# NVIDIA-Merlin/distributed-embeddings

Measured on NVIDIA H100. Metric: DLRM global samples/sec (device-timed, max over ranks), higher is better.
Workload: dtype bf16

## Files before the change

distributed_embeddings_b200/ops/csrc/dense_kernels.cu:

```cuda
#include <cuda_bf16.h>
#include <cuda_runtime.h>
#include <stdint.h>

#include <cstdlib>

#include "common.cuh"
#include "de_b200.h"

namespace de {

namespace {

using bf16 = __nv_bfloat16;

__device__ __forceinline__ uint32_t smem_u32(const void* p) {
  return static_cast<uint32_t>(__cvta_generic_to_shared(p));
}

__device__ __forceinline__ void ldmatrix_x4(uint32_t (&r)[4], uint32_t addr) {
  asm volatile("ldmatrix.sync.aligned.m8n8.x4.shared.b16 {%0,%1,%2,%3}, [%4];"
               : "=r"(r[0]), "=r"(r[1]), "=r"(r[2]), "=r"(r[3])
               : "r"(addr));
}
__device__ __forceinline__ void ldmatrix_x4_trans(uint32_t (&r)[4], uint32_t addr) {
  asm volatile("ldmatrix.sync.aligned.m8n8.x4.trans.shared.b16 {%0,%1,%2,%3}, [%4];"
               : "=r"(r[0]), "=r"(r[1]), "=r"(r[2]), "=r"(r[3])
               : "r"(addr));
}
__device__ __forceinline__ void mma_bf16(float (&c)[4], const uint32_t (&a)[4], uint32_t b0,
                                         uint32_t b1) {
  asm volatile(
      "mma.sync.aligned.m16n8k16.row.col.f32.bf16.bf16.f32 {%0,%1,%2,%3}, {%4,%5,%6,%7}, "
      "{%8,%9}, {%0,%1,%2,%3};"
      : "+f"(c[0]), "+f"(c[1]), "+f"(c[2]), "+f"(c[3])
      : "r"(a[0]), "r"(a[1]), "r"(a[2]), "r"(a[3]), "r"(b0), "r"(b1));
}

constexpr int kMaxFeat = 32;
constexpr int kWarps = 4;

__host__ __device__ constexpr int fwd_warp_bytes(int d) {
  return (kMaxFeat * (d + 8) * 2 > kMaxFeat * 33 * 4) ? kMaxFeat * (d + 8) * 2 : kMaxFeat * 33 * 4;
}

__device__ __forceinline__ void cp_async16(void* smem_dst, const void* gmem_src) {
  asm volatile("cp.async.cg.shared.global [%0], [%1], 16;" ::"r"(smem_u32(smem_dst)),
               "l"(gmem_src)
               : "memory");
}
__device__ __forceinline__ void cp_async_wait_all() {
  asm volatile("cp.async.commit_group;\ncp.async.wait_group 0;" ::: "memory");
}

template <int D>
__device__ __forceinline__ void stage_features(bf16* sF, int LD, const bf16* bottom,
                                               const bf16* emb, int n_emb, int lane) {
  constexpr int kChunks = D / 8;
  const int total = (n_emb + 1) * kChunks;
#pragma unroll 4
  for (int c = lane; c < total; c += 32) {
    const int row = c / kChunks, ch = c - row * kChunks;
    const bf16* src = row == 0 ? bottom + ch * 8 : emb + (row - 1) * D + ch * 8;
    cp_async16(sF + row * LD + ch * 8, src);
  }
  cp_async_wait_all();
}

template <int D>
__device__ __forceinline__ void zero_pad_rows(bf16* sF, int LD, int n_emb, int lane) {
  constexpr int kChunks = D / 8;
  for (int c = (n_emb + 1) * kChunks + lane; c < kMaxFeat * kChunks; c += 32) {
    const int row = c / kChunks, ch = c - row * kChunks;
    *reinterpret_cast<uint4*>(sF + row * LD + ch * 8) = make_uint4(0, 0, 0, 0);
  }
}

template <int D>
__global__ void __launch_bounds__(kWarps * 32)
interact_fwd_kernel(const bf16* __restrict__ bottom, int64_t bottom_stride,
                    const bf16* __restrict__ emb, int64_t emb_stride, int n_emb,
                    bf16* __restrict__ z, int64_t z_stride, int z_width, int64_t batch,
                    const __grid_constant__ SyncArgs sync) {
  sync_head(sync);
  constexpr int LD = D + 8;
  constexpr int kWarpBytes = fwd_warp_bytes(D);
  extern __shared__ __align__(16) unsigned char smem_raw[];
  const int warp = threadIdx.x >> 5, lane = threadIdx.x & 31;
  bf16* sF = reinterpret_cast<bf16*>(smem_raw + warp * kWarpBytes);
  float* sC = reinterpret_cast<float*>(sF);
  const int nf = n_emb + 1;
  const int n_inter = nf * (nf - 1) / 2;

  for (int64_t s = static_cast<int64_t>(blockIdx.x) * kWarps + warp; s < batch;
       s += static_cast<int64_t>(gridDim.x) * kWarps) {
    const bf16* bp = bottom + s * bottom_stride;
    zero_pad_rows<D>(sF, LD, n_emb, lane);
    stage_features<D>(sF, LD, bp, emb + s * emb_stride, n_emb, lane);
    __syncwarp();
    float acc0[2][4] = {}, acc1[4][4] = {};
#pragma unroll
    for (int k = 0; k < D; k += 16) {
      uint32_t a0[4], a1[4], b01[4], b23[4];
      const int arow = lane & 15, acol = k + ((lane >> 4) << 3);
      ldmatrix_x4(a0, smem_u32(sF + arow * LD + acol));
      ldmatrix_x4(a1, smem_u32(sF + (16 + arow) * LD + acol));
      const int brow = (lane & 7) + ((lane >> 4) << 3), bcol = k + (((lane >> 3) & 1) << 3);
      ldmatrix_x4(b01, smem_u32(sF + brow * LD + bcol));
      ldmatrix_x4(b23, smem_u32(sF + (16 + brow) * LD + bcol));
      mma_bf16(acc0[0], a0, b01[0], b01[1]);
      mma_bf16(acc0[1], a0, b01[2], b01[3]);
      mma_bf16(acc1[0], a1, b01[0], b01[1]);
      mma_bf16(acc1[1], a1, b01[2], b01[3]);
      mma_bf16(acc1[2], a1, b23[0], b23[1]);
      mma_bf16(acc1[3], a1, b23[2], b23[3]);
    }
    __syncwarp();
    const int cr = lane >> 2, cc = (lane & 3) << 1;
#pragma unroll
    for (int nt = 0; nt < 2; ++nt) {
      sC[cr * 33 + nt * 8 + cc] = acc0[nt][0];
      sC[cr * 33 + nt * 8 + cc + 1] = acc0[nt][1];
      sC[(cr + 8) * 33 + nt * 8 + cc] = acc0[nt][2];
      sC[(cr + 8) * 33 + nt * 8 + cc + 1] = acc0[nt][3];
    }
#pragma unroll
    for (int nt = 0; nt < 4; ++nt) {
      sC[(16 + cr) * 33 + nt * 8 + cc] = acc1[nt][0];
      sC[(16 + cr) * 33 + nt * 8 + cc + 1] = acc1[nt][1];
      sC[(24 + cr) * 33 + nt * 8 + cc] = acc1[nt][2];
      sC[(24 + cr) * 33 + nt * 8 + cc + 1] = acc1[nt][3];
    }
    __syncwarp();
    bf16* zp = z + s * z_stride;
    for (int idx = lane; idx < n_inter; idx += 32) {
      int i = static_cast<int>((1.0f + sqrtf(1.0f + 8.0f * idx)) * 0.5f);
      while (i * (i - 1) / 2 > idx) --i;
      while ((i + 1) * i / 2 <= idx) ++i;
      const int j = idx - i * (i - 1) / 2;
      zp[idx] = __float2bfloat16_rn(sC[i * 33 + j]);
    }
    for (int c = lane; c < D; c += 32) zp[n_inter + c] = bp[c];
    for (int c = n_inter + D + lane; c < z_width; c += 32) zp[c] = __float2bfloat16_rn(0.f);
    __syncwarp();
  }
  sync_tail(sync);
}

template <int D>
__global__ void __launch_bounds__(kWarps * 32)
interact_bwd_kernel(const bf16* __restrict__ bottom, int64_t bottom_stride,
                    const bf16* __restrict__ emb, int64_t emb_stride, int n_emb,
                    const bf16* __restrict__ dz, int64_t dz_stride, bf16* __restrict__ dbottom,
                    int64_t dbottom_stride, bf16* __restrict__ demb, int64_t demb_stride,
                    float emb_grad_scale, int64_t batch) {
  constexpr int LD = D + 8;
  constexpr int LDG = 40;
  extern __shared__ __align__(16) unsigned char smem_raw[];
  const int warp = threadIdx.x >> 5, lane = threadIdx.x & 31;
  bf16* sF = reinterpret_cast<bf16*>(smem_raw) + warp * (kMaxFeat * LD + kMaxFeat * LDG);
  bf16* sG = sF + kMaxFeat * LD;
  const int nf = n_emb + 1;
  const int n_inter = nf * (nf - 1) / 2;
  zero_pad_rows<D>(sF, LD, n_emb, lane);

  for (int64_t s = static_cast<int64_t>(blockIdx.x) * kWarps + warp; s < batch;
       s += static_cast<int64_t>(gridDim.x) * kWarps) {
    stage_features<D>(sF, LD, bottom + s * bottom_stride, emb + s * emb_stride, n_emb, lane);
    const bf16* dzp = dz + s * dz_stride;
    for (int c = lane; c < kMaxFeat * LDG / 8; c += 32)
      reinterpret_cast<uint4*>(sG)[c] = make_uint4(0, 0, 0, 0);
    __syncwarp();
    for (int idx = lane; idx < n_inter; idx += 32) {
      int i = static_cast<int>((1.0f + sqrtf(1.0f + 8.0f * idx)) * 0.5f);
      while (i * (i - 1) / 2 > idx) --i;
      while ((i + 1) * i / 2 <= idx) ++i;
      const int j = idx - i * (i - 1) / 2;
      const bf16 v = dzp[idx];
      sG[i * LDG + j] = v;
      sG[j * LDG + i] = v;
    }
    __syncwarp();
    uint32_t ga[2][2][4];
#pragma unroll
    for (int mt = 0; mt < 2; ++mt)
#pragma unroll
      for (int ks = 0; ks < 2; ++ks)
        ldmatrix_x4(ga[mt][ks],
                    smem_u32(sG + (mt * 16 + (lane & 15)) * LDG + ks * 16 + ((lane >> 4) << 3)));
    const int cr = lane >> 2, cc = (lane & 3) << 1;
    bf16* dbp = dbottom + s * dbottom_stride;
    bf16* dep = demb + s * demb_stride;
#pragma unroll 1
    for (int n0 = 0; n0 < D; n0 += 32) {
      float acc[2][4][4] = {};
#pragma unroll
      for (int ks = 0; ks < 2; ++ks) {
        uint32_t b01[4], b23[4];
        const int krow = ks * 16 + (lane & 7) + (((lane >> 3) & 1) << 3);
        const int ncol = n0 + ((lane >> 4) << 3);
        ldmatrix_x4_trans(b01, smem_u32(sF + krow * LD + ncol));
        ldmatrix_x4_trans(b23, smem_u32(sF + krow * LD + ncol + 16));
#pragma unroll
        for (int mt = 0; mt < 2; ++mt) {
          mma_bf16(acc[mt][0], ga[mt][ks], b01[0], b01[1]);
          mma_bf16(acc[mt][1], ga[mt][ks], b01[2], b01[3]);
          mma_bf16(acc[mt][2], ga[mt][ks], b23[0], b23[1]);
          mma_bf16(acc[mt][3], ga[mt][ks], b23[2], b23[3]);
        }
      }
#pragma unroll
      for (int mt = 0; mt < 2; ++mt) {
#pragma unroll
        for (int nt = 0; nt < 4; ++nt) {
#pragma unroll
          for (int half = 0; half < 2; ++half) {
            const int row = mt * 16 + cr + half * 8;
            const int col = n0 + nt * 8 + cc;
            float v0 = acc[mt][nt][half * 2], v1 = acc[mt][nt][half * 2 + 1];
            if (row == 0) {
              v0 += __bfloat162float(dzp[n_inter + col]);
              v1 += __bfloat162float(dzp[n_inter + col + 1]);
              *reinterpret_cast<__nv_bfloat162*>(dbp + col) = __floats2bfloat162_rn(v0, v1);
            } else if (row <= n_emb) {
              *reinterpret_cast<__nv_bfloat162*>(dep + (row - 1) * D + col) =
                  __floats2bfloat162_rn(v0 * emb_grad_scale, v1 * emb_grad_scale);
            }
          }
        }
      }
    }
    __syncwarp();
  }
}

__device__ __forceinline__ void cp_async_commit() {
  asm volatile("cp.async.commit_group;" ::: "memory");
}
template <int N>
__device__ __forceinline__ void cp_async_wait_group() {
  asm volatile("cp.async.wait_group %0;" ::"n"(N) : "memory");
}

constexpr int kDzMax = 512;

template <int D>
__device__ __forceinline__ void issue_sample(bf16* sF, int LD, bf16* sDz, const bf16* bottom,
                                             const bf16* emb, const bf16* dz, int n_emb,
                                             int dz_chunks, int lane) {
  constexpr int kChunks = D / 8;
  const int total = (n_emb + 1) * kChunks;
#pragma unroll 4
  for (int c = lane; c < total; c += 32) {
    const int row = c / kChunks, ch = c - row * kChunks;
    const bf16* src = row == 0 ? bottom + ch * 8 : emb + (row - 1) * D + ch * 8;
    cp_async16(sF + row * LD + ch * 8, src);
  }
  for (int c = lane; c < dz_chunks; c += 32) cp_async16(sDz + c * 8, dz + c * 8);
}

struct ChunkDst {
  unsigned long long base;
  long long stride;
};

__device__ __forceinline__ void prefetch_l2(const void* p) {
  asm volatile("prefetch.global.L2 [%0];" ::"l"(p));
}

template <int D, bool APPLY>
__device__ __forceinline__ void
interact_bwd_v2_body(const bf16* __restrict__ bottom, int64_t bottom_stride,
                     const bf16* __restrict__ emb, int64_t emb_stride, int n_emb,
                     const bf16* __restrict__ dz, int64_t dz_stride, bf16* __restrict__ dbottom,
                     int64_t dbottom_stride, bf16* __restrict__ demb, int64_t demb_stride,
                     float emb_grad_scale, int64_t batch, const GradRoute* __restrict__ routes,
                     int n_routes, const SyncArgs& sync, uint32_t* __restrict__ done_counters,
                     int chunk_rows, const InteractApply& apply) {
  constexpr int LD = D + 8;
  constexpr int LDG = 40;
  constexpr int kWarpElems = 2 * kMaxFeat * LD + 2 * kDzMax + kMaxFeat * LDG;
  constexpr int kRowChunks = D / 8;
  extern __shared__ __align__(16) unsigned char smem_raw[];
  const int warp = threadIdx.x >> 5, lane = threadIdx.x & 31;
  bf16* base = reinterpret_cast<bf16*>(smem_raw) + warp * kWarpElems;
  bf16* sDz0 = base + 2 * kMaxFeat * LD;
  bf16* sG = sDz0 + 2 * kDzMax;
  ChunkDst* sDst = reinterpret_cast<ChunkDst*>(reinterpret_cast<bf16*>(smem_raw) +
                                               kWarps * kWarpElems);
  const int nf = n_emb + 1;
  const int n_inter = nf * (nf - 1) / 2;
  const int dz_chunks = (n_inter + D + 7) >> 3;
  const int n_chunks = n_emb * kRowChunks;
  if (routes == nullptr) {
    for (int c = threadIdx.x; c < n_chunks; c += blockDim.x) {
      sDst[c].base = reinterpret_cast<unsigned long long>(demb + c * 8);
      sDst[c].stride = demb_stride * 2;
    }
  } else {
    for (int r = 0; r < n_routes; ++r) {
      const GradRoute R = routes[r];
      const int c0 = R.src_col >> 3, nc = R.width >> 3;
      for (int c = threadIdx.x; c < nc; c += blockDim.x) {
        sDst[c0 + c].base =
            reinterpret_cast<unsigned long long>(reinterpret_cast<bf16*>(R.dst) + R.dst_col + c * 8);
        sDst[c0 + c].stride = R.dst_stride * 2;
      }
    }
  }
  zero_pad_rows<D>(base, LD, n_emb, lane);
  zero_pad_rows<D>(base + kMaxFeat * LD, LD, n_emb, lane);
  __syncthreads();

  float apply_scale = 0.f;
  long long id_cur = -1, id_next = -1;
  if constexpr (APPLY) {
    apply_scale = apply.scale;
    if (apply.scale_ptr != nullptr) apply_scale *= *apply.scale_ptr;
  }
  auto load_id = [&](int64_t smp) -> long long {
    if (lane < n_emb && ((apply.mask >> lane) & 1u)) {
      const long long raw = apply.ids64 ? static_cast<const int64_t*>(apply.ids[lane])[smp]
                                        : static_cast<const int32_t*>(apply.ids[lane])[smp];
      const long long id = raw + apply.id_shift[lane];
      if (static_cast<unsigned long long>(id) < static_cast<unsigned long long>(apply.sub_rows[lane]))
        return id;
    }
    return -1;
  };
  auto prefetch_row = [&](long long id) {
    if (id >= 0) {
      const char* row = reinterpret_cast<const char*>(apply.table[lane] +
                                                      (apply.row_base[lane] + id) * D);
#pragma unroll
      for (int l = 0; l < D * 4 / 128; ++l) prefetch_l2(row + (l << 7));
    }
  };

  const int64_t stride = static_cast<int64_t>(gridDim.x) * kWarps;
  int64_t s = static_cast<int64_t>(blockIdx.x) * kWarps + warp;
  int cur = 0;
  if (s < batch) {
    issue_sample<D>(base, LD, sDz0, bottom + s * bottom_stride, emb + s * emb_stride,
                    dz + s * dz_stride, n_emb, dz_chunks, lane);
    if constexpr (APPLY) {
      id_cur = load_id(s);
      prefetch_row(id_cur);
    }
  }
  cp_async_commit();
  for (; s < batch; s += stride, cur ^= 1) {
    const int64_t nxt = s + stride;
    if (nxt < batch) {
      issue_sample<D>(base + (cur ^ 1) * (kMaxFeat * LD), LD, sDz0 + (cur ^ 1) * kDzMax,
                      bottom + nxt * bottom_stride, emb + nxt * emb_stride, dz + nxt * dz_stride,
                      n_emb, dz_chunks, lane);
      if constexpr (APPLY) id_next = load_id(nxt);
    } else if constexpr (APPLY) {
      id_next = -1;
    }
    cp_async_commit();
    cp_async_wait_group<1>();
    __syncwarp();
    bf16* sF = base + cur * (kMaxFeat * LD);
    const bf16* sDz = sDz0 + cur * kDzMax;
    for (int c = lane; c < kMaxFeat * LDG / 8; c += 32)
      reinterpret_cast<uint4*>(sG)[c] = make_uint4(0, 0, 0, 0);
    __syncwarp();
    for (int idx = lane; idx < n_inter; idx += 32) {
      int i = static_cast<int>((1.0f + sqrtf(1.0f + 8.0f * idx)) * 0.5f);
      while (i * (i - 1) / 2 > idx) --i;
      while ((i + 1) * i / 2 <= idx) ++i;
      const int j = idx - i * (i - 1) / 2;
      const bf16 v = sDz[idx];
      sG[i * LDG + j] = v;
      sG[j * LDG + i] = v;
    }
    __syncwarp();
    uint32_t ga[2][2][4];
#pragma unroll
    for (int mt = 0; mt < 2; ++mt)
#pragma unroll
      for (int ks = 0; ks < 2; ++ks)
        ldmatrix_x4(ga[mt][ks],
                    smem_u32(sG + (mt * 16 + (lane & 15)) * LDG + ks * 16 + ((lane >> 4) << 3)));
    const int cr = lane >> 2, cc = (lane & 3) << 1;
#pragma unroll 1
    for (int n0 = 0; n0 < D; n0 += 32) {
      float acc[2][4][4] = {};
#pragma unroll
      for (int ks = 0; ks < 2; ++ks) {
        uint32_t b01[4], b23[4];
        const int krow = ks * 16 + (lane & 7) + (((lane >> 3) & 1) << 3);
        const int ncol = n0 + ((lane >> 4) << 3);
        ldmatrix_x4_trans(b01, smem_u32(sF + krow * LD + ncol));
        ldmatrix_x4_trans(b23, smem_u32(sF + krow * LD + ncol + 16));
#pragma unroll
        for (int mt = 0; mt < 2; ++mt) {
          mma_bf16(acc[mt][0], ga[mt][ks], b01[0], b01[1]);
          mma_bf16(acc[mt][1], ga[mt][ks], b01[2], b01[3]);
          mma_bf16(acc[mt][2], ga[mt][ks], b23[0], b23[1]);
          mma_bf16(acc[mt][3], ga[mt][ks], b23[2], b23[3]);
        }
      }
#pragma unroll
      for (int mt = 0; mt < 2; ++mt) {
#pragma unroll
        for (int nt = 0; nt < 4; ++nt) {
#pragma unroll
          for (int half = 0; half < 2; ++half) {
            const int row = mt * 16 + cr + half * 8;
            const int col = n0 + nt * 8 + cc;
            float v0 = acc[mt][nt][half * 2], v1 = acc[mt][nt][half * 2 + 1];
            if (row == 0) {
              v0 += __bfloat162float(sDz[n_inter + col]);
              v1 += __bfloat162float(sDz[n_inter + col + 1]);
            } else {
              v0 *= emb_grad_scale;
              v1 *= emb_grad_scale;
            }
            if (row <= n_emb)
              *reinterpret_cast<__nv_bfloat162*>(sF + row * LD + col) =
                  __floats2bfloat162_rn(v0, v1);
          }
        }
      }
    }
    __syncwarp();
    if constexpr (APPLY) prefetch_row(id_next);
    if (lane < kRowChunks)
      *reinterpret_cast<uint4*>(dbottom + s * dbottom_stride + lane * 8) =
          *reinterpret_cast<const uint4*>(sF + lane * 8);
    if constexpr (APPLY) {
      for (int c0 = 0; c0 < n_chunks; c0 += 32) {
        const int c = c0 + lane;
        const int f = c / kRowChunks, ch = c - f * kRowChunks;
        const long long id = __shfl_sync(0xffffffffu, id_cur, f & 31);
        if (c >= n_chunks) continue;
        const uint4 v = *reinterpret_cast<const uint4*>(sF + (f + 1) * LD + ch * 8);
        if ((apply.mask >> f) & 1u) {
          if (id >= 0) {
            const __nv_bfloat162* h = reinterpret_cast<const __nv_bfloat162*>(&v);
            FVec<4> lo, hi;
#pragma unroll
            for (int k = 0; k < 2; ++k) {
              const float2 a = __bfloat1622float2(h[k]), b = __bfloat1622float2(h[k + 2]);
              lo.v[2 * k] = a.x * apply_scale;
              lo.v[2 * k + 1] = a.y * apply_scale;
              hi.v[2 * k] = b.x * apply_scale;
              hi.v[2 * k + 1] = b.y * apply_scale;
            }
            float* dst = apply.table[f] + (apply.row_base[f] + id) * D + ch * 8;
            red_add_f32<4>(dst, lo);
            red_add_f32<4>(dst + 4, hi);
          }
        } else {
          const ChunkDst d = sDst[c];
          *reinterpret_cast<uint4*>(d.base + static_cast<unsigned long long>(s * d.stride)) = v;
        }
      }
      id_cur = id_next;
    } else {
      for (int c = lane; c < n_chunks; c += 32) {
        const int row = 1 + c / kRowChunks, ch = c - (row - 1) * kRowChunks;
        const ChunkDst d = sDst[c];
        *reinterpret_cast<uint4*>(d.base + static_cast<unsigned long long>(s * d.stride)) =
            *reinterpret_cast<const uint4*>(sF + row * LD + ch * 8);
      }
    }
    __syncwarp();
    if (done_counters != nullptr && lane == 0) {
      __threadfence();
      atomicAdd(done_counters + s / chunk_rows, 1u);
    }
  }
  cp_async_wait_group<0>();
  sync_tail(sync);
}

template <int D>
__global__ void __launch_bounds__(kWarps * 32)
interact_bwd_v2_kernel(const bf16* __restrict__ bottom, int64_t bottom_stride,
                       const bf16* __restrict__ emb, int64_t emb_stride, int n_emb,
                       const bf16* __restrict__ dz, int64_t dz_stride, bf16* __restrict__ dbottom,
                       int64_t dbottom_stride, bf16* __restrict__ demb, int64_t demb_stride,
                       float emb_grad_scale, int64_t batch,
                       const GradRoute* __restrict__ routes, int n_routes,
                       const __grid_constant__ SyncArgs sync, uint32_t* __restrict__ done_counters,
                       int chunk_rows) {
  interact_bwd_v2_body<D, false>(bottom, bottom_stride, emb, emb_stride, n_emb, dz, dz_stride,
                                 dbottom, dbottom_stride, demb, demb_stride, emb_grad_scale, batch,
                                 routes, n_routes, sync, done_counters, chunk_rows,
                                 InteractApply{});
}

template <int D>
__global__ void __launch_bounds__(kWarps * 32)
interact_bwd_apply_kernel(const bf16* __restrict__ bottom, int64_t bottom_stride,
                          const bf16* __restrict__ emb, int64_t emb_stride, int n_emb,
                          const bf16* __restrict__ dz, int64_t dz_stride,
                          bf16* __restrict__ dbottom, int64_t dbottom_stride,
                          bf16* __restrict__ demb, int64_t demb_stride, float emb_grad_scale,
                          int64_t batch, const GradRoute* __restrict__ routes, int n_routes,
                          const __grid_constant__ SyncArgs sync,
                          const __grid_constant__ InteractApply apply) {
  interact_bwd_v2_body<D, true>(bottom, bottom_stride, emb, emb_stride, n_emb, dz, dz_stride,
                                dbottom, dbottom_stride, demb, demb_stride, emb_grad_scale, batch,
                                routes, n_routes, sync, nullptr, 0, apply);
}

constexpr int kRbUnroll = 4;
__global__ void __launch_bounds__(256)
relu_bwd_bias_kernel(bf16* __restrict__ dy, const bf16* __restrict__ y, float* __restrict__ db,
                     int64_t rows, int cols, int rows_per_block) {
  extern __shared__ float s_part[];
  const int tpr = cols >> 3;
  const int rows_par = blockDim.x / tpr;
  const int tr = threadIdx.x / tpr, tc = threadIdx.x - tr * tpr;
  const int64_t r0 = static_cast<int64_t>(blockIdx.x) * rows_per_block;
  const int64_t r1 = min(rows, r0 + rows_per_block);
  float acc[8] = {0, 0, 0, 0, 0, 0, 0, 0};
  if (tr < rows_par) {
    for (int64_t r = r0 + tr; r < r1; r += static_cast<int64_t>(rows_par) * kRbUnroll) {
      uint4 g[kRbUnroll], a[kRbUnroll];
#pragma unroll
      for (int u = 0; u < kRbUnroll; ++u) {
        const int64_t rr = r + static_cast<int64_t>(u) * rows_par;
        if (rr < r1) {
          g[u] = *reinterpret_cast<const uint4*>(dy + rr * cols + tc * 8);
          a[u] = *reinterpret_cast<const uint4*>(y + rr * cols + tc * 8);
        }
      }
#pragma unroll
      for (int u = 0; u < kRbUnroll; ++u) {
        const int64_t rr = r + static_cast<int64_t>(u) * rows_par;
        if (rr < r1) {
          uint32_t* gw = reinterpret_cast<uint32_t*>(&g[u]);
          const uint32_t* aw = reinterpret_cast<const uint32_t*>(&a[u]);
#pragma unroll
          for (int i = 0; i < 4; ++i) {
            float2 gf = __bfloat1622float2(*reinterpret_cast<__nv_bfloat162*>(&gw[i]));
            const float2 af = __bfloat1622float2(*reinterpret_cast<const __nv_bfloat162*>(&aw[i]));
            gf.x = af.x > 0.f ? gf.x : 0.f;
            gf.y = af.y > 0.f ? gf.y : 0.f;
            acc[2 * i] += gf.x;
            acc[2 * i + 1] += gf.y;
            __nv_bfloat162 h = __floats2bfloat162_rn(gf.x, gf.y);
            gw[i] = *reinterpret_cast<uint32_t*>(&h);
          }
          *reinterpret_cast<uint4*>(dy + rr * cols + tc * 8) = g[u];
        }
      }
    }
#pragma unroll
    for (int i = 0; i < 8; ++i) s_part[tr * cols + tc * 8 + i] = acc[i];
  }
  __syncthreads();
  for (int c = threadIdx.x; c < cols; c += blockDim.x) {
    float v = 0.f;
    for (int t = 0; t < rows_par; ++t) v += s_part[t * cols + c];
    atomicAdd(db + c, v);
  }
}

__device__ __forceinline__ void unpack8(const uint4& v, float (&f)[8]) {
  const uint32_t* w = reinterpret_cast<const uint32_t*>(&v);
#pragma unroll
  for (int i = 0; i < 4; ++i) {
    const float2 t = unpack2<bf16>(w[i]);
    f[2 * i] = t.x;
    f[2 * i + 1] = t.y;
  }
}
__device__ __forceinline__ uint4 pack8(const float (&f)[8]) {
  uint4 v;
  uint32_t* w = reinterpret_cast<uint32_t*>(&v);
#pragma unroll
  for (int i = 0; i < 4; ++i) w[i] = pack2<bf16>(f[2 * i], f[2 * i + 1]);
  return v;
}

__global__ void __launch_bounds__(256)
cross_fwd_kernel(const uint4* __restrict__ x0, const uint4* __restrict__ s,
                 const uint4* __restrict__ xl, uint4* __restrict__ out, int64_t n_vec) {
  for (int64_t i = static_cast<int64_t>(blockIdx.x) * blockDim.x + threadIdx.x; i < n_vec;
       i += static_cast<int64_t>(gridDim.x) * blockDim.x) {
    float a[8], b[8], c[8];
    unpack8(x0[i], a);
    unpack8(s[i], b);
    unpack8(xl[i], c);
#pragma unroll
    for (int k = 0; k < 8; ++k) c[k] = fmaf(a[k], b[k], c[k]);
    out[i] = pack8(c);
  }
}


__global__ void __launch_bounds__(256)
cross_bwd_kernel(const bf16* __restrict__ dy, const bf16* __restrict__ x0, bf16* __restrict__ g,
                 float* __restrict__ db, int64_t rows, int cols, int tile, int rows_per_block) {
  extern __shared__ float s_part[];
  const int tpr = cols >> 3;
  const int v0 = blockIdx.y * tile;
  const int tw = min(tile, tpr - v0);
  const int rows_par = blockDim.x / tile;
  const int tr = threadIdx.x / tile, tc = threadIdx.x - tr * tile;
  const int64_t r0 = static_cast<int64_t>(blockIdx.x) * rows_per_block;
  const int64_t r1 = min(rows, r0 + rows_per_block);
  float acc[8] = {0, 0, 0, 0, 0, 0, 0, 0};
  const bool active = tr < rows_par && tc < tw;
  if (active) {
    const int64_t col = static_cast<int64_t>(v0 + tc) * 8;
    for (int64_t r = r0 + tr; r < r1; r += static_cast<int64_t>(rows_par) * kRbUnroll) {
      uint4 a[kRbUnroll], b[kRbUnroll];
#pragma unroll
      for (int u = 0; u < kRbUnroll; ++u) {
        const int64_t rr = r + static_cast<int64_t>(u) * rows_par;
        if (rr < r1) {
          a[u] = *reinterpret_cast<const uint4*>(dy + rr * cols + col);
          b[u] = *reinterpret_cast<const uint4*>(x0 + rr * cols + col);
        }
      }
#pragma unroll
      for (int u = 0; u < kRbUnroll; ++u) {
        const int64_t rr = r + static_cast<int64_t>(u) * rows_par;
        if (rr < r1) {
          float fa[8], fb[8];
          unpack8(a[u], fa);
          unpack8(b[u], fb);
#pragma unroll
          for (int k = 0; k < 8; ++k) {
            fa[k] *= fb[k];
            acc[k] += fa[k];
          }
          *reinterpret_cast<uint4*>(g + rr * cols + col) = pack8(fa);
        }
      }
    }
  }
  if (tr < rows_par) {
#pragma unroll
    for (int k = 0; k < 8; ++k) s_part[tr * tile * 8 + tc * 8 + k] = acc[k];
  }
  __syncthreads();
  for (int c = threadIdx.x; c < tw * 8; c += blockDim.x) {
    float v = 0.f;
    for (int t = 0; t < rows_par; ++t) v += s_part[t * tile * 8 + c];
    atomicAdd(db + v0 * 8 + c, v);
  }
}

__global__ void __launch_bounds__(256)
cross_dx0_kernel(const bf16* __restrict__ d_chain, const __grid_constant__ CrossTerms terms,
                 bf16* __restrict__ dx0, bf16* __restrict__ d_bottom, int64_t rows, int cols,
                 int emb_cols, int tile, int rows_per_block) {
  const int tpr = cols >> 3;
  const int v0 = blockIdx.y * tile;
  const int tw = min(tile, tpr - v0);
  const int rows_par = blockDim.x / tile;
  const int tr = threadIdx.x / tile, tc = threadIdx.x - tr * tile;
  if (tr >= rows_par || tc >= tw) return;
  const int col = (v0 + tc) * 8;
  const int64_t r0 = static_cast<int64_t>(blockIdx.x) * rows_per_block;
  const int64_t r1 = min(rows, r0 + rows_per_block);
  const int bcols = cols - emb_cols;
  bf16* dst = col < emb_cols ? dx0 + col : d_bottom + (col - emb_cols);
  const int64_t dst_stride = col < emb_cols ? cols : bcols;
  for (int64_t r = r0 + tr; r < r1; r += rows_par) {
    const int64_t off = r * cols + col;
    float acc[8];
    unpack8(*reinterpret_cast<const uint4*>(d_chain + off), acc);
    for (int l = 0; l < terms.n; ++l) {
      float a[8], b[8];
      unpack8(*(reinterpret_cast<const uint4*>(terms.dy[l]) + off / 8), a);
      unpack8(*(reinterpret_cast<const uint4*>(terms.s[l]) + off / 8), b);
#pragma unroll
      for (int k = 0; k < 8; ++k) acc[k] = fmaf(a[k], b[k], acc[k]);
    }
    *reinterpret_cast<uint4*>(dst + r * dst_stride) = pack8(acc);
  }
}

template <int PL>
__global__ void __launch_bounds__(256)
head_loss_kernel(const bf16* __restrict__ x, int K, const bf16* __restrict__ w,
                 const bf16* __restrict__ bias, const float* __restrict__ labels, int64_t batch,
                 float inv_batch, bf16* __restrict__ dx, float* __restrict__ dw,
                 float* __restrict__ db, float* __restrict__ dbias_prev,
                 float* __restrict__ loss_sum, float* __restrict__ logits_out) {
  extern __shared__ float sred[];
  float* s_dw = sred;
  float* s_dbp = sred + K;
  float* s_misc = sred + 2 * K;
  for (int i = threadIdx.x; i < 2 * K + 2; i += blockDim.x) sred[i] = 0.f;
  __syncthreads();
  const int warp = threadIdx.x >> 5, lane = threadIdx.x & 31;
  const int wpb = blockDim.x >> 5;
  constexpr int per_lane = PL;
  const float b0 = __bfloat162float(bias[0]);
  float wreg[PL];
#pragma unroll
  for (int i = 0; i < PL; ++i) wreg[i] = __bfloat162float(w[lane + 32 * i]);
  float dw_acc[PL], dbp_acc[PL];
#pragma unroll
  for (int i = 0; i < PL; ++i) dw_acc[i] = dbp_acc[i] = 0.f;
  float loss_acc = 0.f, db_acc = 0.f;
  for (int64_t s = static_cast<int64_t>(blockIdx.x) * wpb + warp; s < batch;
       s += static_cast<int64_t>(gridDim.x) * wpb) {
    float xv[PL];
    float dot = 0.f;
#pragma unroll
    for (int i = 0; i < PL; ++i) {
      if (i < per_lane) {
        xv[i] = __bfloat162float(x[s * K + lane + 32 * i]);
        dot = fmaf(xv[i], wreg[i], dot);
      }
    }
#pragma unroll
    for (int off = 16; off > 0; off >>= 1) dot += __shfl_xor_sync(0xffffffffu, dot, off);
    const float logit = dot + b0;
    const float label = labels[s];
    const float loss = fmaxf(logit, 0.f) - logit * label + log1pf(__expf(-fabsf(logit)));
    const float sig = 1.f / (1.f + __expf(-logit));
    const float dl = (sig - label) * inv_batch;
    if (lane == 0) {
      loss_acc += loss;
      db_acc += dl;
      if (logits_out) logits_out[s] = logit;
    }
#pragma unroll
    for (int i = 0; i < PL; ++i) {
      if (i < per_lane) {
        dw_acc[i] = fmaf(dl, xv[i], dw_acc[i]);
        const float g = xv[i] > 0.f ? dl * wreg[i] : 0.f;
        dbp_acc[i] += g;
        dx[s * K + lane + 32 * i] = __float2bfloat16_rn(g);
      }
    }
  }
#pragma unroll
  for (int i = 0; i < PL; ++i) {
    if (i < per_lane) {
      atomicAdd(&s_dw[lane + 32 * i], dw_acc[i]);
      atomicAdd(&s_dbp[lane + 32 * i], dbp_acc[i]);
    }
  }
  if (lane == 0) {
    atomicAdd(&s_misc[0], loss_acc);
    atomicAdd(&s_misc[1], db_acc);
  }
  __syncthreads();
  for (int i = threadIdx.x; i < K; i += blockDim.x) {
    atomicAdd(dw + i, s_dw[i]);
    atomicAdd(dbias_prev + i, s_dbp[i]);
  }
  if (threadIdx.x == 0) {
    atomicAdd(loss_sum, s_misc[0] * inv_batch);
    atomicAdd(db, s_misc[1]);
  }
}

template <int PL>
__global__ void __launch_bounds__(256)
head_eval_kernel(const bf16* __restrict__ x, const bf16* __restrict__ w,
                 const bf16* __restrict__ bias, const float* __restrict__ labels, int64_t batch,
                 const int64_t* __restrict__ n_valid, float* __restrict__ probs,
                 unsigned long long* __restrict__ hist, int nb, double* __restrict__ loss_sum,
                 unsigned long long* __restrict__ count) {
  constexpr int K = 32 * PL;
  __shared__ float s_loss;
  if (threadIdx.x == 0) s_loss = 0.f;
  __syncthreads();
  const int warp = threadIdx.x >> 5, lane = threadIdx.x & 31;
  const int wpb = blockDim.x >> 5;
  int64_t nv = *n_valid;
  nv = nv < 0 ? 0 : (nv > batch ? batch : nv);
  const float b0 = __bfloat162float(bias[0]);
  const float nbf = static_cast<float>(nb);
  float wreg[PL];
#pragma unroll
  for (int i = 0; i < PL; ++i) wreg[i] = __bfloat162float(w[lane + 32 * i]);
  float loss_acc = 0.f;
  for (int64_t g0 = (static_cast<int64_t>(blockIdx.x) * wpb + warp) * 32; g0 < batch;
       g0 += static_cast<int64_t>(gridDim.x) * wpb * 32) {
    const int rows = batch - g0 < 32 ? static_cast<int>(batch - g0) : 32;
    float my_logit = 0.f;
#pragma unroll 4
    for (int j = 0; j < rows; ++j) {
      const bf16* xr = x + (g0 + j) * K;
      float dot = 0.f;
#pragma unroll
      for (int i = 0; i < PL; ++i) dot = fmaf(__bfloat162float(xr[lane + 32 * i]), wreg[i], dot);
#pragma unroll
      for (int off = 16; off > 0; off >>= 1) dot += __shfl_xor_sync(0xffffffffu, dot, off);
      if (lane == j) my_logit = dot + b0;
    }
    const int64_t s = g0 + lane;
    const bool has_row = lane < rows;
    const bool valid = s < nv;
    const float logit = my_logit;
    const float p = 1.f / (1.f + __expf(-logit));
    if (has_row) probs[s] = p;
    int key = -1;
    if (valid) {
      const float label = labels[s];
      loss_acc += fmaxf(logit, 0.f) - logit * label + log1pf(__expf(-fabsf(logit)));
      int k = static_cast<int>(ceilf(__fmul_rn(p, nbf))) - 1;
      k = k < 0 ? 0 : (k > nb - 1 ? nb - 1 : k);
      key = (label > 0.5f ? nb : 0) + k;
    }
    const unsigned peers = __match_any_sync(0xffffffffu, key);
    if (key >= 0 && lane == __ffs(peers) - 1)
      atomicAdd(hist + key, static_cast<unsigned long long>(__popc(peers)));
  }
#pragma unroll
  for (int off = 16; off > 0; off >>= 1) loss_acc += __shfl_xor_sync(0xffffffffu, loss_acc, off);
  if (lane == 0) atomicAdd(&s_loss, loss_acc);
  __syncthreads();
  if (threadIdx.x == 0) {
    atomicAdd(loss_sum, static_cast<double>(s_loss));
    if (blockIdx.x == 0) atomicAdd(count, static_cast<unsigned long long>(nv));
  }
}

__global__ void __launch_bounds__(256)
sgd_update_kernel(float* __restrict__ p32, bf16* __restrict__ p16, float* __restrict__ g32,
                  const float* __restrict__ lr_ptr, float grad_scale, int64_t n_vec4) {
  const float step = -(*lr_ptr) * grad_scale;
  const int64_t stride = static_cast<int64_t>(gridDim.x) * blockDim.x;
  for (int64_t i = static_cast<int64_t>(blockIdx.x) * blockDim.x + threadIdx.x; i < n_vec4;
       i += stride) {
    float4 p = reinterpret_cast<float4*>(p32)[i];
    const float4 g = reinterpret_cast<const float4*>(g32)[i];
    p.x = fmaf(step, g.x, p.x);
    p.y = fmaf(step, g.y, p.y);
    p.z = fmaf(step, g.z, p.z);
    p.w = fmaf(step, g.w, p.w);
    reinterpret_cast<float4*>(p32)[i] = p;
    reinterpret_cast<float4*>(g32)[i] = make_float4(0.f, 0.f, 0.f, 0.f);
    __nv_bfloat162 a = __floats2bfloat162_rn(p.x, p.y), b = __floats2bfloat162_rn(p.z, p.w);
    uint2 o;
    o.x = *reinterpret_cast<uint32_t*>(&a);
    o.y = *reinterpret_cast<uint32_t*>(&b);
    reinterpret_cast<uint2*>(p16)[i] = o;
  }
}

template <int KIND>
__device__ __forceinline__ void dense_opt_elem(float& p, float& a, float& v, float g, float lr,
                                               float beta1, float beta2, float bias1, float bias2,
                                               float eps) {
  if constexpr (KIND == kOptAdagrad) {
    a = fmaf(g, g, a);
    p -= lr * g / (sqrtf(a) + eps);
  } else {
    a = beta1 * a + (1.f - beta1) * g;
    v = beta2 * v + (1.f - beta2) * g * g;
    const float mh = a / bias1;
    const float vh = v / bias2;
    p -= lr * mh / (sqrtf(vh) + eps);
  }
}

template <int KIND>
__global__ void __launch_bounds__(256)
dense_opt_kernel(float* __restrict__ p32, bf16* __restrict__ p16, float* __restrict__ g32,
                 float* __restrict__ s0, float* __restrict__ s1, const float* __restrict__ lr_ptr,
                 const float* __restrict__ step_ptr, float beta1, float beta2, float eps,
                 int64_t n_vec4) {
  const float lr = *lr_ptr;
  float bias1 = 1.f, bias2 = 1.f;
  if constexpr (KIND == kOptAdam) {
    const float t = *step_ptr;
    bias1 = 1.f - powf(beta1, t);
    bias2 = 1.f - powf(beta2, t);
  }
  const int64_t stride = static_cast<int64_t>(gridDim.x) * blockDim.x;
  for (int64_t i = static_cast<int64_t>(blockIdx.x) * blockDim.x + threadIdx.x; i < n_vec4;
       i += stride) {
    float4 p = reinterpret_cast<float4*>(p32)[i];
    const float4 g = reinterpret_cast<const float4*>(g32)[i];
    float4 a = reinterpret_cast<float4*>(s0)[i];
    float4 v = make_float4(0.f, 0.f, 0.f, 0.f);
    if constexpr (KIND == kOptAdam) v = reinterpret_cast<float4*>(s1)[i];
    dense_opt_elem<KIND>(p.x, a.x, v.x, g.x, lr, beta1, beta2, bias1, bias2, eps);
    dense_opt_elem<KIND>(p.y, a.y, v.y, g.y, lr, beta1, beta2, bias1, bias2, eps);
    dense_opt_elem<KIND>(p.z, a.z, v.z, g.z, lr, beta1, beta2, bias1, bias2, eps);
    dense_opt_elem<KIND>(p.w, a.w, v.w, g.w, lr, beta1, beta2, bias1, bias2, eps);
    reinterpret_cast<float4*>(p32)[i] = p;
    reinterpret_cast<float4*>(s0)[i] = a;
    if constexpr (KIND == kOptAdam) reinterpret_cast<float4*>(s1)[i] = v;
    reinterpret_cast<float4*>(g32)[i] = make_float4(0.f, 0.f, 0.f, 0.f);
    __nv_bfloat162 lo = __floats2bfloat162_rn(p.x, p.y), hi = __floats2bfloat162_rn(p.z, p.w);
    uint2 o;
    o.x = *reinterpret_cast<uint32_t*>(&lo);
    o.y = *reinterpret_cast<uint32_t*>(&hi);
    reinterpret_cast<uint2*>(p16)[i] = o;
  }
}

__global__ void cast_pad_kernel(const float* __restrict__ src, int src_cols, bf16* __restrict__ dst,
                                int dst_cols, int64_t rows) {
  const int64_t n = rows * dst_cols;
  const int64_t stride = static_cast<int64_t>(gridDim.x) * blockDim.x;
  for (int64_t i = static_cast<int64_t>(blockIdx.x) * blockDim.x + threadIdx.x; i < n;
       i += stride) {
    const int64_t r = i / dst_cols;
    const int c = static_cast<int>(i - r * dst_cols);
    dst[i] = __float2bfloat16_rn(c < src_cols ? src[r * src_cols + c] : 0.f);
  }
}

__global__ void __launch_bounds__(256)
avgpool_fwd_kernel(const bf16* __restrict__ x, int64_t x_stride, int n, bf16* __restrict__ out,
                   int64_t out_stride, int out_len, int stride, int left, int64_t rows) {
  const int64_t total = rows * out_len;
  const int64_t step = static_cast<int64_t>(gridDim.x) * blockDim.x;
  for (int64_t i = static_cast<int64_t>(blockIdx.x) * blockDim.x + threadIdx.x; i < total;
       i += step) {
    const int64_t r = i / out_len;
    const int j = static_cast<int>(i - r * out_len);
    const int lo = max(0, j * stride - left), hi = min(n, (j + 1) * stride - left);
    const bf16* xp = x + r * x_stride;
    float acc = 0.f;
    for (int c = lo; c < hi; ++c) acc += __bfloat162float(xp[c]);
    out[r * out_stride + j] = __float2bfloat16_rn(hi > lo ? acc / static_cast<float>(hi - lo) : 0.f);
  }
}

__global__ void __launch_bounds__(256)
avgpool_bwd_kernel(const bf16* __restrict__ dout, int64_t dout_stride, int out_len,
                   bf16* __restrict__ dx, int64_t dx_stride, int n, int stride, int left,
                   int64_t rows) {
  const int64_t total = rows * n;
  const int64_t step = static_cast<int64_t>(gridDim.x) * blockDim.x;
  for (int64_t i = static_cast<int64_t>(blockIdx.x) * blockDim.x + threadIdx.x; i < total;
       i += step) {
    const int64_t r = i / n;
    const int c = static_cast<int>(i - r * n);
    const int j = (c + left) / stride;
    const int lo = max(0, j * stride - left), hi = min(n, (j + 1) * stride - left);
    const float g = j < out_len ? __bfloat162float(dout[r * dout_stride + j]) : 0.f;
    dx[r * dx_stride + c] = __float2bfloat16_rn(g / static_cast<float>(hi - lo));
  }
}

}

void launch_avgpool_fwd(const void* x, int64_t x_stride, int n, void* out, int64_t out_stride,
                        int out_len, int stride, int left, int64_t rows, cudaStream_t stream) {
  if (rows <= 0 || out_len <= 0) return;
  int64_t blocks = (rows * out_len + 255) / 256;
  if (blocks > kGridCapSms * 16) blocks = kGridCapSms * 16;
  avgpool_fwd_kernel<<<static_cast<unsigned>(blocks), 256, 0, stream>>>(
      reinterpret_cast<const bf16*>(x), x_stride, n, reinterpret_cast<bf16*>(out), out_stride,
      out_len, stride, left, rows);
}

void launch_avgpool_bwd(const void* dout, int64_t dout_stride, int out_len, void* dx,
                        int64_t dx_stride, int n, int stride, int left, int64_t rows,
                        cudaStream_t stream) {
  if (rows <= 0 || n <= 0) return;
  int64_t blocks = (rows * n + 255) / 256;
  if (blocks > kGridCapSms * 16) blocks = kGridCapSms * 16;
  avgpool_bwd_kernel<<<static_cast<unsigned>(blocks), 256, 0, stream>>>(
      reinterpret_cast<const bf16*>(dout), dout_stride, out_len, reinterpret_cast<bf16*>(dx),
      dx_stride, n, stride, left, rows);
}

bool launch_interact_fwd(const void* bottom, int64_t bottom_stride, const void* emb,
                         int64_t emb_stride, int n_emb, int dim, void* z, int64_t z_stride,
                         int z_width, int64_t batch, int sm_count, cudaStream_t stream,
                         const SyncArgs& sync) {
  if (n_emb + 1 > kMaxFeat || batch <= 0) return false;
  int64_t blocks = (batch + kWarps - 1) / kWarps;
  const int64_t cap = static_cast<int64_t>(sm_count) * 8;
  if (blocks > cap) blocks = cap;
#define DE_IFWD(DD)                                                                              \
  {                                                                                              \
    const size_t smem = kWarps * fwd_warp_bytes(DD);                                             \
    cudaFuncSetAttribute(interact_fwd_kernel<DD>, cudaFuncAttributeMaxDynamicSharedMemorySize,   \
                         static_cast<int>(smem));                                                \
    interact_fwd_kernel<DD><<<static_cast<unsigned>(blocks), kWarps * 32, smem, stream>>>(       \
        reinterpret_cast<const bf16*>(bottom), bottom_stride, reinterpret_cast<const bf16*>(emb), \
        emb_stride, n_emb, reinterpret_cast<bf16*>(z), z_stride, z_width, batch, sync);          \
    return true;                                                                                 \
  }
  if (dim == 128) DE_IFWD(128)
  if (dim == 64) DE_IFWD(64)
  if (dim == 32) DE_IFWD(32)
  if (dim == 16) DE_IFWD(16)
#undef DE_IFWD
  return false;
}

bool launch_interact_bwd(const void* bottom, int64_t bottom_stride, const void* emb,
                         int64_t emb_stride, int n_emb, int dim, const void* dz,
                         int64_t dz_stride, void* dbottom, int64_t dbottom_stride, void* demb,
                         int64_t demb_stride, float emb_grad_scale, int64_t batch, int sm_count,
                         cudaStream_t stream, const GradRoute* routes, int n_routes,
                         const SyncArgs& sync, uint32_t* done_counters, int chunk_rows,
                         const InteractApply* apply) {
  if (n_emb + 1 > kMaxFeat || batch <= 0 || dim % 32 != 0) return false;
  const bool applied = apply != nullptr && apply->mask != 0;
  if (applied && (dim != 128 || done_counters != nullptr)) return false;
  int64_t blocks = (batch + kWarps - 1) / kWarps;
  const int64_t cap = static_cast<int64_t>(sm_count) * 8;
  if (blocks > cap) blocks = cap;
  static const bool force_v1 = [] {
    const char* v = std::getenv("DE_B200_INTERACT_V1");
    return v != nullptr && v[0] == '1';
  }();
  const int nf = n_emb + 1;
  const int dz_elems = (nf * (nf - 1) / 2 + dim + 7) / 8 * 8;
  const bool v2_ok =
      dz_elems <= kDzMax && dz_elems <= dz_stride && dz_stride % 8 == 0 &&
      bottom_stride % 8 == 0 && emb_stride % 8 == 0 && dbottom_stride % 8 == 0 &&
      ((reinterpret_cast<uintptr_t>(dz) | reinterpret_cast<uintptr_t>(bottom) |
        reinterpret_cast<uintptr_t>(emb) | reinterpret_cast<uintptr_t>(dbottom)) & 15) == 0 &&
      (dim == 128 || dim == 64) &&
      (routes != nullptr || (demb_stride % 8 == 0 && (reinterpret_cast<uintptr_t>(demb) & 15) == 0));
  if ((routes != nullptr || done_counters != nullptr || applied) && !v2_ok) return false;
  const bool has_sync = sync.state != nullptr && (sync.wait_ch >= 0 || sync.signal_ch >= 0);
  if (v2_ok &&
      (!force_v1 || routes != nullptr || has_sync || done_counters != nullptr || applied)) {
    int64_t blocks2 = (batch + kWarps - 1) / kWarps;
    if (blocks2 > static_cast<int64_t>(sm_count) * 2) blocks2 = static_cast<int64_t>(sm_count) * 2;
#define DE_IBWD2(KERNEL, DD, ...)                                                                \
  {                                                                                              \
    const size_t smem =                                                                          \
        kWarps * (2 * kMaxFeat * (DD + 8) + 2 * kDzMax + kMaxFeat * 40) * sizeof(bf16) +         \
        static_cast<size_t>(n_emb) * (DD / 8) * sizeof(ChunkDst);                                \
    cudaFuncSetAttribute(KERNEL<DD>, cudaFuncAttributeMaxDynamicSharedMemorySize,                \
                         static_cast<int>(smem));                                                \
    KERNEL<DD><<<static_cast<unsigned>(blocks2), kWarps * 32, smem, stream>>>(                   \
        reinterpret_cast<const bf16*>(bottom), bottom_stride, reinterpret_cast<const bf16*>(emb), \
        emb_stride, n_emb, reinterpret_cast<const bf16*>(dz), dz_stride,                         \
        reinterpret_cast<bf16*>(dbottom), dbottom_stride, reinterpret_cast<bf16*>(demb),         \
        demb_stride, emb_grad_scale, batch, routes, n_routes, sync, __VA_ARGS__);                \
    return true;                                                                                 \
  }
    if (applied) DE_IBWD2(interact_bwd_apply_kernel, 128, *apply)
    if (dim == 128) DE_IBWD2(interact_bwd_v2_kernel, 128, done_counters, chunk_rows)
    if (dim == 64) DE_IBWD2(interact_bwd_v2_kernel, 64, done_counters, chunk_rows)
#undef DE_IBWD2
  }
  if (has_sync) return false;
#define DE_IBWD(DD)                                                                              \
  {                                                                                              \
    const size_t smem = kWarps * (kMaxFeat * (DD + 8) + kMaxFeat * 40) * sizeof(bf16);           \
    cudaFuncSetAttribute(interact_bwd_kernel<DD>, cudaFuncAttributeMaxDynamicSharedMemorySize,   \
                         static_cast<int>(smem));                                                \
    interact_bwd_kernel<DD><<<static_cast<unsigned>(blocks), kWarps * 32, smem, stream>>>(       \
        reinterpret_cast<const bf16*>(bottom), bottom_stride, reinterpret_cast<const bf16*>(emb), \
        emb_stride, n_emb, reinterpret_cast<const bf16*>(dz), dz_stride,                         \
        reinterpret_cast<bf16*>(dbottom), dbottom_stride, reinterpret_cast<bf16*>(demb),         \
        demb_stride, emb_grad_scale, batch);                                                     \
    return true;                                                                                 \
  }
  if (dim == 128) DE_IBWD(128)
  if (dim == 64) DE_IBWD(64)
  if (dim == 32) DE_IBWD(32)
#undef DE_IBWD
  return false;
}

static void cross_tiling(int cols, int* tile, int* n_tiles, int* rows_per_block) {
  const int tpr = cols / 8;
  int best_t = 0, best_n = 0;
  double best = -1.0;
  for (int n = (tpr + 255) / 256; n <= tpr && n <= 64; ++n) {
    const int t = (tpr + n - 1) / n;
    const int rows_par = 256 / t;
    const double busy = static_cast<double>(rows_par * t) / 256.0 *
                        static_cast<double>(tpr) / static_cast<double>(n * t);
    if (busy > best + 1e-9) {
      best = busy;
      best_t = t;
      best_n = n;
    }
  }
  *tile = best_t;
  *n_tiles = best_n;
  *rows_per_block = (256 / best_t) * kRbUnroll * 4;
}

void launch_cross_fwd(const void* x0, const void* s, const void* xl, void* out, int64_t n,
                      int sm_count, cudaStream_t stream) {
  const int64_t n_vec = n / 8;
  if (n_vec <= 0) return;
  int64_t blocks = (n_vec + 255) / 256;
  if (blocks > sm_count * 8) blocks = sm_count * 8;
  cross_fwd_kernel<<<static_cast<unsigned>(blocks), 256, 0, stream>>>(
      reinterpret_cast<const uint4*>(x0), reinterpret_cast<const uint4*>(s),
      reinterpret_cast<const uint4*>(xl), reinterpret_cast<uint4*>(out), n_vec);
}

void launch_cross_bwd(const void* dy, const void* x0, void* g, float* db, int64_t rows, int cols,
                      cudaStream_t stream) {
  if (rows <= 0) return;
  int tile, n_tiles, rpb;
  cross_tiling(cols, &tile, &n_tiles, &rpb);
  const dim3 grid(static_cast<unsigned>((rows + rpb - 1) / rpb), static_cast<unsigned>(n_tiles));
  const size_t smem = static_cast<size_t>(256 / tile) * tile * 8 * sizeof(float);
  cross_bwd_kernel<<<grid, 256, smem, stream>>>(
      reinterpret_cast<const bf16*>(dy), reinterpret_cast<const bf16*>(x0),
      reinterpret_cast<bf16*>(g), db, rows, cols, tile, rpb);
}

void launch_cross_dx0(const void* d_chain, const CrossTerms& terms, void* dx0, void* d_bottom,
                      int64_t rows, int cols, int emb_cols, cudaStream_t stream) {
  if (rows <= 0) return;
  int tile, n_tiles, rpb;
  cross_tiling(cols, &tile, &n_tiles, &rpb);
  const dim3 grid(static_cast<unsigned>((rows + rpb - 1) / rpb), static_cast<unsigned>(n_tiles));
  cross_dx0_kernel<<<grid, 256, 0, stream>>>(
      reinterpret_cast<const bf16*>(d_chain), terms, reinterpret_cast<bf16*>(dx0),
      reinterpret_cast<bf16*>(d_bottom), rows, cols, emb_cols, tile, rpb);
}

void launch_relu_bwd_bias(void* dy, const void* y, float* db, int64_t rows, int cols,
                          cudaStream_t stream) {
  if (rows <= 0) return;
  const int tpr = cols / 8;
  const int threads = 256;
  const int rows_par = threads / tpr;
  const int rows_per_block = rows_par * kRbUnroll * 4;
  const int64_t blocks = (rows + rows_per_block - 1) / rows_per_block;
  const size_t smem = static_cast<size_t>(rows_par) * cols * sizeof(float);
  relu_bwd_bias_kernel<<<static_cast<unsigned>(blocks), threads, smem, stream>>>(
      reinterpret_cast<bf16*>(dy), reinterpret_cast<const bf16*>(y), db, rows, cols,
      rows_per_block);
}

bool launch_head_loss(const void* x, int K, const void* w, const void* bias, const float* labels,
                      int64_t batch, float inv_batch, void* dx, float* dw, float* db,
                      float* dbias_prev, float* loss_sum, float* logits_out, int sm_count,
                      cudaStream_t stream) {
  if (batch <= 0) return true;
  const int threads = 256;
  int64_t blocks = (batch + 7) / 8;
  if (blocks > sm_count * 4) blocks = sm_count * 4;
  const size_t smem = (2 * K + 2) * sizeof(float);
#define DE_HEAD(PL)                                                                              \
  head_loss_kernel<PL><<<static_cast<unsigned>(blocks), threads, smem, stream>>>(                \
      reinterpret_cast<const bf16*>(x), K, reinterpret_cast<const bf16*>(w),                     \
      reinterpret_cast<const bf16*>(bias), labels, batch, inv_batch, reinterpret_cast<bf16*>(dx), \
      dw, db, dbias_prev, loss_sum, logits_out)
  switch (K) {
    case 64: DE_HEAD(2); break;
    case 128: DE_HEAD(4); break;
    case 256: DE_HEAD(8); break;
    case 512: DE_HEAD(16); break;
    case 1024: DE_HEAD(32); break;
    default: return false;
  }
#undef DE_HEAD
  return true;
}

bool launch_head_eval(const void* x, int K, const void* w, const void* bias, const float* labels,
                      int64_t batch, const int64_t* n_valid, float* probs, int64_t* hist, int nb,
                      double* loss_sum, int64_t* count, int sm_count, cudaStream_t stream) {
  if (K != 64 && K != 128 && K != 256 && K != 512 && K != 1024) return false;
  if (batch <= 0) return true;
  const int threads = 256;
  int64_t blocks = (batch + 255) / 256;
  if (blocks > sm_count * 4) blocks = sm_count * 4;
#define DE_HEAD_EVAL(PL)                                                                         \
  head_eval_kernel<PL><<<static_cast<unsigned>(blocks), threads, 0, stream>>>(                  \
      reinterpret_cast<const bf16*>(x), reinterpret_cast<const bf16*>(w),                        \
      reinterpret_cast<const bf16*>(bias), labels, batch, n_valid, probs,                        \
      reinterpret_cast<unsigned long long*>(hist), nb, loss_sum,                                 \
      reinterpret_cast<unsigned long long*>(count))
  switch (K) {
    case 64: DE_HEAD_EVAL(2); break;
    case 128: DE_HEAD_EVAL(4); break;
    case 256: DE_HEAD_EVAL(8); break;
    case 512: DE_HEAD_EVAL(16); break;
    default: DE_HEAD_EVAL(32); break;
  }
#undef DE_HEAD_EVAL
  return true;
}

void launch_sgd_update(float* p32, void* p16, float* g32, const float* lr_ptr, float grad_scale,
                       int64_t n, int sm_count, cudaStream_t stream) {
  const int64_t n_vec4 = n / 4;
  if (n_vec4 <= 0) return;
  int64_t blocks = (n_vec4 + 255) / 256;
  if (blocks > sm_count * 8) blocks = sm_count * 8;
  sgd_update_kernel<<<static_cast<unsigned>(blocks), 256, 0, stream>>>(
      p32, reinterpret_cast<bf16*>(p16), g32, lr_ptr, grad_scale, n_vec4);
}

bool launch_dense_opt(int kind, float* p32, void* p16, float* g32, float* s0, float* s1,
                      const float* lr_ptr, const float* step_ptr, float beta1, float beta2,
                      float eps, int64_t n, int sm_count, cudaStream_t stream) {
  if (kind != kOptAdagrad && kind != kOptAdam) return false;
  const int64_t n_vec4 = n / 4;
  if (n_vec4 <= 0) return true;
  int64_t blocks = (n_vec4 + 255) / 256;
  if (blocks > sm_count * 8) blocks = sm_count * 8;
  if (kind == kOptAdagrad)
    dense_opt_kernel<kOptAdagrad><<<static_cast<unsigned>(blocks), 256, 0, stream>>>(
        p32, reinterpret_cast<bf16*>(p16), g32, s0, nullptr, lr_ptr, nullptr, 0.f, 0.f, eps,
        n_vec4);
  else
    dense_opt_kernel<kOptAdam><<<static_cast<unsigned>(blocks), 256, 0, stream>>>(
        p32, reinterpret_cast<bf16*>(p16), g32, s0, s1, lr_ptr, step_ptr, beta1, beta2, eps,
        n_vec4);
  return true;
}

void launch_cast_pad(const float* src, int src_cols, void* dst, int dst_cols, int64_t rows,
                     cudaStream_t stream) {
  if (rows <= 0) return;
  int64_t blocks = (rows * dst_cols + 255) / 256;
  if (blocks > kGridCapSms * 8) blocks = kGridCapSms * 8;
  cast_pad_kernel<<<static_cast<unsigned>(blocks), 256, 0, stream>>>(
      src, src_cols, reinterpret_cast<bf16*>(dst), dst_cols, rows);
}

}
```

Before: 17.92 million.

## Double-buffer interaction forward loads and vectorize output stores via smem staging

The dot-interaction forward kernel now double-buffers feature tiles in shared memory, prefetching the next sample with cp.async while computing the current one. Results are written directly into a packed bf16 shared output row (lower triangle plus bottom features) and then stored to global memory with 16-byte vector writes instead of scattered per-element writes that needed an inverse-triangular index computation. The grid size now comes from occupancy queries rather than a fixed 8 blocks per SM. This roughly doubles shared memory per warp and adds a fixed cap on output row width (kZMax) that is not checked at launch.

```diff
diff --git a/distributed_embeddings_b200/ops/csrc/dense_kernels.cu b/distributed_embeddings_b200/ops/csrc/dense_kernels.cu
--- a/distributed_embeddings_b200/ops/csrc/dense_kernels.cu
+++ b/distributed_embeddings_b200/ops/csrc/dense_kernels.cu
@@ -38,9 +38,10 @@
 
 constexpr int kMaxFeat = 32;
 constexpr int kWarps = 4;
+constexpr int kZMax = 640;
 
 __host__ __device__ constexpr int fwd_warp_bytes(int d) {
-  return (kMaxFeat * (d + 8) * 2 > kMaxFeat * 33 * 4) ? kMaxFeat * (d + 8) * 2 : kMaxFeat * 33 * 4;
+  return 2 * kMaxFeat * (d + 8) * 2 + kZMax * 2;
 }
 
 __device__ __forceinline__ void cp_async16(void* smem_dst, const void* gmem_src) {
@@ -51,9 +52,16 @@
 __device__ __forceinline__ void cp_async_wait_all() {
   asm volatile("cp.async.commit_group;\ncp.async.wait_group 0;" ::: "memory");
 }
+__device__ __forceinline__ void cp_async_commit() {
+  asm volatile("cp.async.commit_group;" ::: "memory");
+}
+template <int N>
+__device__ __forceinline__ void cp_async_wait_group() {
+  asm volatile("cp.async.wait_group %0;" ::"n"(N) : "memory");
+}
 
 template <int D>
-__device__ __forceinline__ void stage_features(bf16* sF, int LD, const bf16* bottom,
+__device__ __forceinline__ void issue_features(bf16* sF, int LD, const bf16* bottom,
                                                const bf16* emb, int n_emb, int lane) {
   constexpr int kChunks = D / 8;
   const int total = (n_emb + 1) * kChunks;
@@ -63,8 +71,16 @@
     const bf16* src = row == 0 ? bottom + ch * 8 : emb + (row - 1) * D + ch * 8;
     cp_async16(sF + row * LD + ch * 8, src);
   }
+}
+
+template <int D>
+__device__ __forceinline__ void stage_features(bf16* sF, int LD, const bf16* bottom,
+                                               const bf16* emb, int n_emb, int lane) {
+  issue_features<D>(sF, LD, bottom, emb, n_emb, lane);
   cp_async_wait_all();
 }
+
+__device__ __forceinline__ int tri(int i) { return i * (i - 1) / 2; }
 
 template <int D>
 __device__ __forceinline__ void zero_pad_rows(bf16* sF, int LD, int n_emb, int lane) {
@@ -83,20 +99,40 @@
                     const __grid_constant__ SyncArgs sync) {
   sync_head(sync);
   constexpr int LD = D + 8;
-  constexpr int kWarpBytes = fwd_warp_bytes(D);
+  constexpr int kBuf = kMaxFeat * LD;
   extern __shared__ __align__(16) unsigned char smem_raw[];
   const int warp = threadIdx.x >> 5, lane = threadIdx.x & 31;
-  bf16* sF = reinterpret_cast<bf16*>(smem_raw + warp * kWarpBytes);
-  float* sC = reinterpret_cast<float*>(sF);
+  bf16* base = reinterpret_cast<bf16*>(smem_raw + warp * fwd_warp_bytes(D));
+  bf16* sZ = base + 2 * kBuf;
   const int nf = n_emb + 1;
   const int n_inter = nf * (nf - 1) / 2;
-
-  for (int64_t s = static_cast<int64_t>(blockIdx.x) * kWarps + warp; s < batch;
-       s += static_cast<int64_t>(gridDim.x) * kWarps) {
-    const bf16* bp = bottom + s * bottom_stride;
-    zero_pad_rows<D>(sF, LD, n_emb, lane);
-    stage_features<D>(sF, LD, bp, emb + s * emb_stride, n_emb, lane);
+  const int n_valid = n_inter + D;
+  const int n_vec = (n_valid + 7) >> 3;
+  const bool vec = ((reinterpret_cast<uintptr_t>(z) & 15) == 0) && (z_stride & 7) == 0;
+  const bf16 zero = __float2bfloat16_rn(0.f);
+  zero_pad_rows<D>(base, LD, n_emb, lane);
+  zero_pad_rows<D>(base + kBuf, LD, n_emb, lane);
+  for (int c = n_valid + lane; c < n_vec * 8; c += 32) sZ[c] = zero;
+  const int cr = lane >> 2, cc = (lane & 3) << 1;
+  auto put = [&](int i, int j, float v) {
+    if (j < i && i < nf) sZ[tri(i) + j] = __float2bfloat16_rn(v);
+  };
+
+  const int64_t stride = static_cast<int64_t>(gridDim.x) * kWarps;
+  int64_t s = static_cast<int64_t>(blockIdx.x) * kWarps + warp;
+  int cur = 0;
+  if (s < batch)
+    issue_features<D>(base, LD, bottom + s * bottom_stride, emb + s * emb_stride, n_emb, lane);
+  cp_async_commit();
+  for (; s < batch; s += stride, cur ^= 1) {
+    const int64_t nxt = s + stride;
+    if (nxt < batch)
+      issue_features<D>(base + (cur ^ 1) * kBuf, LD, bottom + nxt * bottom_stride,
+                        emb + nxt * emb_stride, n_emb, lane);
+    cp_async_commit();
+    cp_async_wait_group<1>();
     __syncwarp();
+    const bf16* sF = base + cur * kBuf;
     float acc0[2][4] = {}, acc1[4][4] = {};
 #pragma unroll
     for (int k = 0; k < D; k += 16) {
@@ -114,35 +150,35 @@
       mma_bf16(acc1[2], a1, b23[0], b23[1]);
       mma_bf16(acc1[3], a1, b23[2], b23[3]);
     }
-    __syncwarp();
-    const int cr = lane >> 2, cc = (lane & 3) << 1;
 #pragma unroll
     for (int nt = 0; nt < 2; ++nt) {
-      sC[cr * 33 + nt * 8 + cc] = acc0[nt][0];
-      sC[cr * 33 + nt * 8 + cc + 1] = acc0[nt][1];
-      sC[(cr + 8) * 33 + nt * 8 + cc] = acc0[nt][2];
-      sC[(cr + 8) * 33 + nt * 8 + cc + 1] = acc0[nt][3];
+      put(cr, nt * 8 + cc, acc0[nt][0]);
+      put(cr, nt * 8 + cc + 1, acc0[nt][1]);
+      put(cr + 8, nt * 8 + cc, acc0[nt][2]);
+      put(cr + 8, nt * 8 + cc + 1, acc0[nt][3]);
     }
 #pragma unroll
     for (int nt = 0; nt < 4; ++nt) {
-      sC[(16 + cr) * 33 + nt * 8 + cc] = acc1[nt][0];
-      sC[(16 + cr) * 33 + nt * 8 + cc + 1] = acc1[nt][1];
-      sC[(24 + cr) * 33 + nt * 8 + cc] = acc1[nt][2];
-      sC[(24 + cr) * 33 + nt * 8 + cc + 1] = acc1[nt][3];
-    }
+      put(16 + cr, nt * 8 + cc, acc1[nt][0]);
+      put(16 + cr, nt * 8 + cc + 1, acc1[nt][1]);
+      put(24 + cr, nt * 8 + cc, acc1[nt][2]);
+      put(24 + cr, nt * 8 + cc + 1, acc1[nt][3]);
+    }
+    for (int c = lane; c < D; c += 32) sZ[n_inter + c] = sF[c];
     __syncwarp();
     bf16* zp = z + s * z_stride;
-    for (int idx = lane; idx < n_inter; idx += 32) {
-      int i = static_cast<int>((1.0f + sqrtf(1.0f + 8.0f * idx)) * 0.5f);
-      while (i * (i - 1) / 2 > idx) --i;
-      while ((i + 1) * i / 2 <= idx) ++i;
-      const int j = idx - i * (i - 1) / 2;
-      zp[idx] = __float2bfloat16_rn(sC[i * 33 + j]);
-    }
-    for (int c = lane; c < D; c += 32) zp[n_inter + c] = bp[c];
-    for (int c = n_inter + D + lane; c < z_width; c += 32) zp[c] = __float2bfloat16_rn(0.f);
+    int c0 = 0;
+    if (vec) {
+      const int full = z_width >> 3;
+      for (int c = lane; c < full; c += 32)
+        *reinterpret_cast<uint4*>(zp + c * 8) =
+            c < n_vec ? *reinterpret_cast<const uint4*>(sZ + c * 8) : make_uint4(0, 0, 0, 0);
+      c0 = full * 8;
+    }
+    for (int c = c0 + lane; c < z_width; c += 32) zp[c] = c < n_valid ? sZ[c] : zero;
     __syncwarp();
   }
+  cp_async_wait_group<0>();
   sync_tail(sync);
 }
 
@@ -231,14 +267,6 @@
     }
     __syncwarp();
   }
-}
-
-__device__ __forceinline__ void cp_async_commit() {
-  asm volatile("cp.async.commit_group;" ::: "memory");
-}
-template <int N>
-__device__ __forceinline__ void cp_async_wait_group() {
-  asm volatile("cp.async.wait_group %0;" ::"n"(N) : "memory");
 }
 
 constexpr int kDzMax = 512;
@@ -967,19 +995,34 @@
       dx_stride, n, stride, left, rows);
 }
 
+template <typename Kernel>
+static int resident_blocks(Kernel kernel, int threads, size_t smem) {
+  cudaFuncSetAttribute(kernel, cudaFuncAttributeMaxDynamicSharedMemorySize, static_cast<int>(smem));
+  int n = 0;
+  if (cudaOccupancyMaxActiveBlocksPerMultiprocessor(&n, kernel, threads, smem) != cudaSuccess)
+    return 0;
+  return n;
+}
+
+static int64_t wave_blocks(int64_t batch, int warps, int per_sm, int sm_count) {
+  const int64_t blocks = (batch + warps - 1) / warps;
+  const int64_t wave = static_cast<int64_t>(per_sm) * sm_count;
+  return blocks < wave ? blocks : wave;
+}
+
 bool launch_interact_fwd(const void* bottom, int64_t bottom_stride, const void* emb,
                          int64_t emb_stride, int n_emb, int dim, void* z, int64_t z_stride,
                          int z_width, int64_t batch, int sm_count, cudaStream_t stream,
                          const SyncArgs& sync) {
   if (n_emb + 1 > kMaxFeat || batch <= 0) return false;
-  int64_t blocks = (batch + kWarps - 1) / kWarps;
-  const int64_t cap = static_cast<int64_t>(sm_count) * 8;
-  if (blocks > cap) blocks = cap;
 #define DE_IFWD(DD)                                                                              \
   {                                                                                              \
     const size_t smem = kWarps * fwd_warp_bytes(DD);                                             \
+    static const int per_sm = resident_blocks(interact_fwd_kernel<DD>, kWarps * 32, smem);       \
+    if (per_sm < 1) return false;                                                                \
     cudaFuncSetAttribute(interact_fwd_kernel<DD>, cudaFuncAttributeMaxDynamicSharedMemorySize,   \
                          static_cast<int>(smem));                                                \
+    const int64_t blocks = wave_blocks(batch, kWarps, per_sm, sm_count);                         \
     interact_fwd_kernel<DD><<<static_cast<unsigned>(blocks), kWarps * 32, smem, stream>>>(       \
         reinterpret_cast<const bf16*>(bottom), bottom_stride, reinterpret_cast<const bf16*>(emb), \
         emb_stride, n_emb, reinterpret_cast<bf16*>(z), z_stride, z_width, batch, sync);          \
```

Result: faster. 18.16 million (median of 6 runs) (+1.3%).
